# torgeiba/CPUPerformanceRayTracer

Measured on AMD Instinct MI355X. Metric: ray-samples/sec (pixels×spp×bounces) at 1920×1080; ms/frame, higher is better.
Workload: dtype f32; 1 GPU; c2_1080p; width=1920, height=1080, spp=8, bounces=8, parallelism=single GPU, step=one launch accumulating 8 frames (spp) of every pixel in HBM

## Files before the change

### cpuperformanceraytracer_amd/csrc/pt_chain.h

```cpp
#pragma once
#include <hip/hip_runtime.h>
#include <stdint.h>

#include "pt_kernel.h"
#include "pt_guard.h"
#include "pt_tile_queue.h"

__device__ __forceinline__ float pt_px_ld(const float* p)
{
    return __builtin_bit_cast(float, __hip_atomic_load(reinterpret_cast<uint32_t*>(const_cast<float*>(p)), __ATOMIC_RELAXED,
                                                       __HIP_MEMORY_SCOPE_AGENT));
}
__device__ __forceinline__ void pt_px_st(float* p, float v)
{
    __hip_atomic_store(reinterpret_cast<uint32_t*>(p), __builtin_bit_cast(uint32_t, v), __ATOMIC_RELAXED, __HIP_MEMORY_SCOPE_AGENT);
}

typedef unsigned pt_v3u __attribute__((ext_vector_type(3)));
typedef float pt_v3f __attribute__((ext_vector_type(3)));
constexpr int kPtCpolSc1 = 16;
constexpr int kPtBufRsrcWord3 = 0x00020000;
__device__ __forceinline__ void pt_px_ld3(const float* buf, uint32_t nbytes, size_t cs, size_t pi, float& x, float& y, float& z)
{
    if (cs == 1 && nbytes) {
        const __amdgpu_buffer_rsrc_t r = __builtin_amdgcn_make_buffer_rsrc(const_cast<float*>(buf), 0, (int)nbytes, kPtBufRsrcWord3);
        const pt_v3f v = __builtin_bit_cast(pt_v3f, __builtin_amdgcn_raw_buffer_load_b96(r, (int)(pi * 4u), 0, kPtCpolSc1));
        x = v.x, y = v.y, z = v.z;
        return;
    }
    x = pt_px_ld(buf + pi), y = pt_px_ld(buf + pi + cs), z = pt_px_ld(buf + pi + 2 * cs);
}
__device__ __forceinline__ void pt_px_st3(float* buf, uint32_t nbytes, size_t cs, size_t pi, float x, float y, float z)
{
    if (cs == 1 && nbytes) {
        const __amdgpu_buffer_rsrc_t r = __builtin_amdgcn_make_buffer_rsrc(buf, 0, (int)nbytes, kPtBufRsrcWord3);
        const pt_v3f v = {x, y, z};
        __builtin_amdgcn_raw_buffer_store_b96(__builtin_bit_cast(pt_v3u, v), r, (int)(pi * 4u), 0, kPtCpolSc1);
        return;
    }
    pt_px_st(buf + pi, x), pt_px_st(buf + pi + cs, y), pt_px_st(buf + pi + 2 * cs, z);
}
__device__ __forceinline__ uint32_t pt_px_nbytes(size_t floats)
{
    return floats * 4u < (1ull << 31) ? (uint32_t)(floats * 4u) : 0u;
}

__device__ __forceinline__ void pt_chain_started(unsigned long long* started)
{
    if (started && threadIdx.x == 0) __hip_atomic_fetch_add(started, 1ull, __ATOMIC_RELAXED, __HIP_MEMORY_SCOPE_SYSTEM);
}

__device__ __forceinline__ bool pt_chain_ready(const uint32_t* ep, uint32_t e, uint32_t w)
{
    const uint32_t t = pt_entry_tile(e), part = pt_entry_part(e);
    uint32_t m = ~0u;
    if (part != 2u) {
        const uint32_t a = __hip_atomic_load(const_cast<uint32_t*>(ep + 2u * t), __ATOMIC_RELAXED, __HIP_MEMORY_SCOPE_AGENT);
        m = a < m ? a : m;
    }
    if (part != 1u) {
        const uint32_t b = __hip_atomic_load(const_cast<uint32_t*>(ep + 2u * t + 1u), __ATOMIC_RELAXED, __HIP_MEMORY_SCOPE_AGENT);
        m = b < m ? b : m;
    }
    return __builtin_amdgcn_readfirstlane(m) >= w;
}

#ifndef PT_CHAIN_DIAG
#define PT_CHAIN_DIAG 0
#endif
constexpr uint32_t kPtChainPolls = PT_CHAIN_DIAG ? 1u << 16 : 1u << 21;
static __device__ uint32_t pt_chain_polls_dev = kPtChainPolls;
constexpr uint32_t kPtDiagWaves = 34, kPtDiagEnded = 35, kPtDiagWaiting = 36;
__device__ __forceinline__ unsigned* pt_chain_diag_prev(unsigned* q, uint32_t seq)
{
    return q - (size_t)(seq % 4u) * PT_QUEUE_WORDS + (size_t)((seq + 3u) % 4u) * PT_QUEUE_WORDS;
}
__device__ __forceinline__ void pt_chain_wait(const uint32_t* ep, uint32_t e, uint32_t w, uint32_t* err, int lane,
                                              unsigned* qdiag = nullptr)
{
    if (pt_chain_ready(ep, e, w)) return;
    bool ok = false;
    uint32_t polls = 0;
    if (PT_CHAIN_DIAG && qdiag && lane == 0) atomicAdd(qdiag + kPtDiagWaiting, 1u);
    do {
        __builtin_amdgcn_s_sleep(8);
        ok = pt_chain_ready(ep, e, w);
    } while (!ok && ++polls < pt_chain_polls_dev);
    if (PT_CHAIN_DIAG && qdiag && lane == 0) atomicSub(qdiag + kPtDiagWaiting, 1u);
#if PT_CHAIN_DIAG
    if (!ok && lane == 0 && qdiag) {
        unsigned* const qp = pt_chain_diag_prev(qdiag, w + 1u);
        auto rd = [](unsigned* p) { return __hip_atomic_fetch_add(p, 0u, __ATOMIC_RELAXED, __HIP_MEMORY_SCOPE_AGENT); };
        const uint32_t t = pt_entry_tile(e);
        printf("chain wait ran out: launch %u entry %u (tile %u) epochs %u %u | this launch: waves %u ended %u waiting %u "
               "| previous: waves %u ended %u waiting %u | block %u wave %u\n",
               w + 1u, e, t, rd(const_cast<uint32_t*>(ep + 2u * t)), rd(const_cast<uint32_t*>(ep + 2u * t + 1u)),
               rd(qdiag + kPtDiagWaves), rd(qdiag + kPtDiagEnded), rd(qdiag + kPtDiagWaiting), rd(qp + kPtDiagWaves),
               rd(qp + kPtDiagEnded), rd(qp + kPtDiagWaiting), blockIdx.x, threadIdx.x >> 6);
    }
#endif
    if (!ok && lane == 0) {
        const uint32_t t = pt_entry_tile(e), part = pt_entry_part(e);
        uint32_t m = ~0u;
        if (part != 2u) m = __hip_atomic_fetch_add(const_cast<uint32_t*>(ep + 2u * t), 0u, __ATOMIC_RELAXED, __HIP_MEMORY_SCOPE_AGENT);
        if (part != 1u) {
            const uint32_t b = __hip_atomic_fetch_add(const_cast<uint32_t*>(ep + 2u * t + 1u), 0u, __ATOMIC_RELAXED, __HIP_MEMORY_SCOPE_AGENT);
            m = b < m ? b : m;
        }
        const uint32_t behind = m >= w ? 0u : (w - m < 127u ? w - m : 127u);
        pt_guard_report(err, PT_G_CHAIN_WAIT, (t & 0xffffffu) | (behind << 24) | (m < w ? 0x80000000u : 0u));
    }
}

__device__ __forceinline__ void pt_chain_publish(uint32_t* ep, uint32_t e, uint32_t seq, uint32_t delay, int lane)
{
    if (__builtin_expect(delay != 0u, 0)) {
        const unsigned long long t0 = __builtin_amdgcn_s_memrealtime();
        while (__builtin_amdgcn_s_memrealtime() - t0 < 100ull * delay) __builtin_amdgcn_s_sleep(8);
    }
    asm volatile("s_waitcnt vmcnt(0)" ::: "memory");
    if (lane == 0) {
        const uint32_t t = pt_entry_tile(e), part = pt_entry_part(e);
        if (part != 2u) __hip_atomic_store(ep + 2u * t, seq, __ATOMIC_RELAXED, __HIP_MEMORY_SCOPE_AGENT);
        if (part != 1u) __hip_atomic_store(ep + 2u * t + 1u, seq, __ATOMIC_RELAXED, __HIP_MEMORY_SCOPE_AGENT);
    }
}
```

### cpuperformanceraytracer_amd/csrc/pt_guard.h

```cpp
#pragma once
#include <hip/hip_runtime.h>
#include <stdint.h>

#include "pt_kernel.h"

#ifndef PT_CHECKED
#define PT_CHECKED 0
#endif

__device__ __forceinline__ void pt_guard_report(uint32_t* err, uint32_t id, uint32_t detail)
{
    if (!err) return;
    atomicAdd(&err[PT_ERR_GUARD_COUNT], 1u);
    atomicMin(reinterpret_cast<unsigned long long*>(err + PT_ERR_GUARD_FIRST), ((unsigned long long)id << 32) | detail);
}

#define PT_GUARD(err, cond, id, detail) \
    (!PT_CHECKED || (cond) || (pt_guard_report((err), (uint32_t)(id), (uint32_t)(detail)), false))
```

### cpuperformanceraytracer_amd/csrc/pt_kernel.hip

```cpp
#include "pt_kernel.h"
#include "pt_exactmath.h"
#include "pt_sincosf.h"
#define PT_IT_HD __device__ __forceinline__
#define PT_IT_DIV(a, b) pt::div_guarded((a), (b))
#define PT_IT_SQRT(x) pt::sqrt_guarded(x)
#include "pt_invtrig.h"
#define PT_EC_HD __device__ __forceinline__
#define PT_EC_RCP(x) pt::rcp_rn(x)
#define PT_EC_DIV(a, b) pt::div_rn((a), (b), pt::rcp_rn(b))
#define PT_EC_SQRT(x) pt::sqrt_rn(x)
#include "pt_envcert.h"
#include "pt_tile_queue.h"
#include "pt_kernel_pick.h"
#include "pt_guard.h"
#include "pt_tonemap.h"
#include "pt_output.h"
#include "pt_wave.h"
#include "pt_chain.h"
#include <math.h>
#include <algorithm>
#include <utility>

namespace {

// ... 761 lines not shown
                    next_item += ntaken;
                }
                if ((live & ~idle) == 0 && ntaken == 0) break;
                ++tile_work;
                DIAG_ADD(1, t_it);
                DIAG_MARK(t_dir);
                if (COUNT) ++n_iter;
                bool queued = false;
                if (had || took) {
                    D = normalize(add(n, random_unit_vector(rng)));
                    DIAG_ADD(2, t_dir);
                    DIAG_MARK(t_tr);
                    const Hit h = trace<DemofoxScene, false, QV, SPHC>(s_axis, s_qv, P, D);
                    DIAG_ADD(3, t_tr);
                    DIAG_MARK(t_sh);
                    if (COUNT) ++n_seg, n_fb += (unsigned long long)h.fb;
                    bool done;
                    if (h.best == PT_SUPER_FAR) {
                        if (DEFER) queued = true;
                        else ret = add(ret, miss_radiance<ENV>(job, amb, D));
                        done = true;
                        if (COUNT) ++n_esc;
                    } else {
                        const PtLdsPrim pr = prim_at(s_prim, h.id);
                        n = hit_normal(pr, h, P, D);
                        P = add(add(P, mul(D, h.best)), mul(n, PT_NUDGE));
                        ret = add(ret, mulv(v3(pr.er, pr.eg, pr.eb), T));
                        T = mulv(T, v3(pr.ar, pr.ag, pr.ab));
                        bounce += 1;
                        done = bounce > B;
                    }
                    if (done) {
                        if (own && it_f == nf - 1) {
                            c_keep = ret;
                        } else {
                            lds_f32* c = col_lds + (it_lane * CHS + it_f) * 3;
                            c[0] = ret.x;
                            c[1] = ret.y;
                            c[2] = ret.z;
                        }
                        bounce = 0;
                    }
                    DIAG_ADD(4, t_sh);
                }
                if (DEFER) {
                    const uint64_t qm = pt_ballot(queued);
                    if (queued) {
                        const int r = __builtin_amdgcn_mbcnt_hi((uint32_t)(qm >> 32),
                                                               __builtin_amdgcn_mbcnt_lo((uint32_t)qm, 0u));
                        envq[qn + r] = make_float4(D.x, D.y, D.z, __builtin_bit_cast(float, (it_lane * CHS + it_f) * 3));
                    }
                    qn += __popcll(qm);
                    if (qn >= 64) {
                        qn -= 64;
                        drain(qn, 64);
                    }
                }
            }
            if (DEFER && qn > 0) drain(0, qn);
            if (f0 + CH >= S) next_tile = tq.next(job.err);
            DIAG_MARK(t_c);
            const int clc = txi * 8 + (lane & 7), clr = tyi * 8 + (lane >> 3);
            const bool cvalid = clc < job.ncols && clr < job.nrows && pt_part_has_lane(part, lane);
            if (cvalid) {
                if (!MULTI) {
                    const float* px = job.buf + out_index<LAYOUT>(job, clc, clr);
                    acc = v3(px[0], px[cs], px[2 * cs]);
                }
                for (int fi = 0; fi < nf; ++fi) {
                    V3 c = c_keep;
                    if (mine) {
                        if (own && fi == nf - 1) {
                            c = c_keep;
                        } else {
                            const lds_f32* cp = col_lds + (lane * CHS + fi) * 3;
                            c = v3(cp[0], cp[1], cp[2]);
                        }
                    }
                    const V3 colr = c;
                    const int f = f0 + fi;
                    const float t = WTAB && f < kMaxWeights ? s_w[f] : pt::rcp_rn((float)(job.frame_first + (uint32_t)f) + 1.0f);
                    acc = add(acc, mul(sub(colr, acc), t));
                }
            }
            DIAG_ADD(5, t_c);
        }
        }
        if (txi * 8 + (lane & 7) < job.ncols && tyi * 8 + (lane >> 3) < job.nrows && pt_part_has_lane(part, lane)) {
            float* px = job.buf + out_index<LAYOUT>(job, txi * 8 + (lane & 7), tyi * 8 + (lane >> 3));
            px[0] = acc.x;
            px[cs] = acc.y;
            px[2 * cs] = acc.z;
        }
        if (job.cost && lane == 0) pt_record_cost(job.cost, this_tile, total_tiles, tile_work);
        if (S <= 0) next_tile = tq.next(job.err);
        tile = __builtin_amdgcn_readfirstlane(next_tile);
#if PT_DIAG && !PT_DIAG_WAVES_ONLY
        if (job.counters && lane == 0 && n_tiles_diag <= 32) {
            unsigned long long* tl = job.counters + 32 + 4 * 65536 + 96 * (size_t)(blockIdx.x * kWavesPerBlock + wv);
            tl[3 * (n_tiles_diag - 1) + 0] = r_tile0;
            tl[3 * (n_tiles_diag - 1) + 1] = __builtin_amdgcn_s_memrealtime();
            tl[3 * (n_tiles_diag - 1) + 2] = ((unsigned long long)diag_tile_id << 32) | tile_work;
        }
#endif
        DIAG_ADD(6, t_tile);
    }
    tq.report(job.err);
    if (COUNT) {
        for (int off = 32; off > 0; off >>= 1) {
            n_seg += __shfl_xor(n_seg, off, 64);
            n_samp += __shfl_xor(n_samp, off, 64);
            n_esc += __shfl_xor(n_esc, off, 64);
            n_prim += __shfl_xor(n_prim, off, 64);
            n_fb += __shfl_xor(n_fb, off, 64);
            n_sky += __shfl_xor(n_sky, off, 64);
        }
        if (lane == 0) {
            atomicAdd(&job.counters[PT_CNT_SEGMENTS], n_seg);
            atomicAdd(&job.counters[PT_CNT_LANE_SLOTS], 64ull * n_iter);
            atomicAdd(&job.counters[PT_CNT_SAMPLES], n_samp);
            atomicAdd(&job.counters[PT_CNT_ESCAPED], n_esc);
            atomicAdd(&job.counters[PT_CNT_PRIMARY], n_prim);
            atomicAdd(&job.counters[PT_CNT_FALLBACK], n_fb);
            atomicAdd(&job.counters[PT_CNT_SKY], n_sky);
        }
    }
#if PT_DIAG
    if (job.counters && lane == 0) {
#if PT_DIAG >= 2
            for (int k = 0; k < 7; ++k) atomicAdd(&job.counters[PT_CNT_N + k], dg[k]);
#endif
            const unsigned long long r_death = __builtin_amdgcn_s_memrealtime();
#if !PT_DIAG_NOATOMIC
            const unsigned long long t_death = __builtin_amdgcn_s_memtime();
            atomicAdd(&job.counters[PT_CNT_N + 7], t_death - t_birth);
            atomicAdd(&job.counters[PT_CNT_N + 10], r_death - r_birth);
            atomicMax(&job.counters[PT_CNT_N + 8], r_birth);
            atomicMin(&job.counters[PT_CNT_N + 9], r_death);
            atomicMax(&job.counters[PT_CNT_N + 11], r_death);
            atomicMin(&job.counters[PT_CNT_N + 12], r_birth);
#endif
            unsigned long long* rec = job.counters + 32 + 4 * (size_t)(blockIdx.x * kWavesPerBlock + wv);
            rec[0] = r_birth;
            rec[1] = r_death;
            rec[2] = n_tiles_diag;
            rec[3] = n_iter;
    }
#endif
}

constexpr uint32_t kCtWaveFloats = 2u * 64u * (uint32_t)kChunk * 3u;
enum : int {
    kWsTcur, kWsHm, kWsHm1, kWsNh, kWsF0next, kWsF0A, kWsTD, kWsF0D, kWsNfD, kWsHmD, kWsHmD1,
    kWsTileSeg, kWsSegA, kWsSegD, kWsFlags, kWsChunks, kWsCamMode, kWsCam, kWsCam1, kWsWords
};

#ifndef PT_ENV_WAVES
#define PT_ENV_WAVES 6
#endif
#ifndef PT_ENV_Q
#define PT_ENV_Q 96
#endif
static_assert(PT_ENV_Q >= 64 && PT_ENV_Q <= 128, "the env miss queue holds 64 .. 128 entries per wave");
template <int LAYOUT, bool ENV, bool COUNT, bool PRESENT>
__device__ __forceinline__ void render_body_ct(const PtJob& job)
{
    pt_chain_started(job.started);
#if PT_CHAIN_DIAG
    if (job.tile_epoch && blockIdx.x == 0 && threadIdx.x == 0) job.queue[kPtDiagWaves] = gridDim.x * (blockDim.x / 64u);
#endif
    const PtScene* __restrict__ sc = job.scene;
    constexpr int kWavesPerBlock = waves_per_block<ENV>();
    constexpr bool QV = true;
    __shared__ PtLdsPrim s_prim[PT_NPRIMS];
    __shared__ AxisRow s_axis[PT_NQUADS * kAxisRowsPerQuad<true>];
    __shared__ float4 s_qv[kQuadVecs];
    __shared__ float s_w[kMaxWeights];
    __shared__ float4 s_rec[kWavesPerBlock][64];
    __shared__ float s_nrm[kWavesPerBlock][3][64];
    __shared__ float s_acc[kWavesPerBlock][3][64];
    __shared__ uint32_t s_seed[kWavesPerBlock][64];
    __shared__ uint32_t s_ws[kWavesPerBlock][kWsWords];
    __shared__ uint32_t s_tq[kWavesPerBlock][PtTileQueue<kWavesPerBlock>::kWords];
    constexpr int kQ = ENV ? PT_ENV_Q : 1;
    __shared__ float4 s_envq[ENV ? kWavesPerBlock : 1][kQ][2];
    {
        const int t = threadIdx.x;
        if (t < PT_NPRIMS) {
            PtLdsPrim e;
            if (t < PT_NQUADS) {
                e.nx = sc->qn[t][0]; e.ny = sc->qn[t][1]; e.nz = sc->qn[t][2];
            } else {
                e.nx = sc->sph[t - PT_NQUADS][0]; e.ny = sc->sph[t - PT_NQUADS][1]; e.nz = sc->sph[t - PT_NQUADS][2];
            }
            e.ar = sc->albedo[t][0]; e.ag = sc->albedo[t][1]; e.ab = sc->albedo[t][2];
            e.er = sc->emissive[t][0]; e.eg = sc->emissive[t][1]; e.eb = sc->emissive[t][2];
            e.pad0 = e.pad1 = e.pad2 = 0.0f;
            s_prim[t] = e;
        } else if (t >= 64 && t < 64 + PT_NQUADS * kAxisRowsPerQuad<true>) {
            constexpr int F = kAxisRowsPerQuad<true> / 3;
            const int r = (t - 64) / 3, k = (t - 64) % 3, q = r / F, fl = r % F;
            const auto vk = [&](int v) { return sc->qv[q][fl ? 3 - v : v][k]; };
            s_axis[t - 64] = AxisRow{vk(0), vk(1), vk(2), vk(3)};
        } else if (t >= 128 && t < 128 + kQuadVecs) {
            const int r = (t - 128) / 3, part = (t - 128) % 3, q = r >> 1, fl = r & 1;
            float e[4];
            for (int i = 0; i < 4; ++i) {
                const int f = part * 4 + i, v = f / 3, k = f % 3;
                e[i] = sc->qv[q][fl ? 3 - v : v][k];
            }
            s_qv[t - 128] = make_float4(e[0], e[1], e[2], e[3]);
        }
        if (t < kMaxWeights && t < job.nframes)
            s_w[t] = pt::rcp_rn((float)(job.frame_first + (uint32_t)t) + 1.0f);
    }
    __syncthreads();

    const int lane = threadIdx.x & 63;
    const int wv = __builtin_amdgcn_readfirstlane(threadIdx.x >> 6);
    const int tiles_x = (job.ncols + 7) >> 3;
    const uint32_t total_tiles = (uint32_t)tiles_x * (uint32_t)((job.nrows + 7) >> 3);
    const int S = job.nframes, B = job.num_bounces;
    const size_t cs = (LAYOUT == PT_LAYOUT_INTERLEAVED) ? 1u : 8u;
    float* const slots = job.ct_slots + (size_t)(blockIdx.x * kWavesPerBlock + wv) * kCtWaveFloats;
    if (!PT_GUARD(job.err, blockIdx.x * (uint32_t)kWavesPerBlock + (uint32_t)wv < job.ct_waves, PT_G_SLOT_BASE,
                  blockIdx.x * (uint32_t)kWavesPerBlock + (uint32_t)wv))
        return;
    const size_t px_extent = pixel_extent<LAYOUT>(job);
    const uint32_t pxb = pt_px_nbytes(px_extent);
    auto weight = [&](int f) {
        return f < kMaxWeights ? s_w[f] : pt::rcp_rn((float)(job.frame_first + (uint32_t)f) + 1.0f);
    };
    auto present = [&](int lc, int lr, const V3& acc) {
        if constexpr (PRESENT) {
            const size_t o = (size_t)lr * (uint32_t)job.ncols + (uint32_t)lc;
            if (PT_GUARD(job.err, o < (size_t)job.nrows * (uint32_t)job.ncols, PT_G_PIXOUT, o))
                job.pix_out[o] = pt_tone::pack<true, true>(acc.x, acc.y, acc.z, job.pix_xrgb != 0);
        }
    };

    Camera cam;
    cam.W = job.cam_W;
    cam.H = job.cam_H;
    cam.yW = job.cam_yW;
    cam.yH = job.cam_yH;
    cam.aspect = job.cam_aspect;
    cam.yAspect = job.cam_yAspect;
    cam.cam_dist = sc->cam_dist;
    const V3 amb = v3(sc->ambient[0], sc->ambient[1], sc->ambient[2]);
    const V3 zero = v3(0.0f, 0.0f, 0.0f), one = v3(1.0f, 1.0f, 1.0f);
    unsigned long long n_seg = 0, n_iter = 0, n_samp = 0, n_esc = 0, n_prim = 0, n_fb = 0, n_sky = 0, n_cam = 0;
#if PT_DIAG
    const unsigned long long r_birth = __builtin_amdgcn_s_memrealtime();
    unsigned long long n_tiles_diag = 0;
    uint32_t didx_cur = 0, didxA = 0, didxD = 0;
    unsigned long long* const dtl =
        job.counters ? job.counters + 32 + 4 * 65536 + 96 * (size_t)(blockIdx.x * kWavesPerBlock + wv) : nullptr;
#endif

    pt_queue_zero_next(job.queue_next);
    constexpr uint32_t kNone = PtTileQueue<kWavesPerBlock>::kNone;
    {
        PtTileQueue<kWavesPerBlock> q(job.queue, job.order, job.units, job.nunits, total_tiles, wv);
        q.back = (uint64_t)blockIdx.x * 100u >= (uint64_t)gridDim.x * (100u - (job.ct_back_pct < 100u ? job.ct_back_pct : 100u)) &&
                 job.ct_back_pct != 0;
        q.save(s_tq[wv], lane);
    }

    uint32_t* const ws = s_ws[wv];
    auto ws_ld = [&](int k) -> uint32_t { return __builtin_amdgcn_readfirstlane(ws[k]); };
    auto ws_st = [&](int k, uint32_t v) {
        if (lane == 0) ws[k] = v;
    };
    auto chain_wait_tile = [&](uint32_t e) {
        if (job.chain_wait != 0u) pt_chain_wait(job.tile_epoch, e, job.chain_wait, job.err, lane, PT_CHAIN_DIAG ? job.queue : nullptr);
    };
    auto chain_publish = [&](uint32_t e) {
        if (job.tile_epoch) pt_chain_publish(job.tile_epoch, e, job.chain_seq, job.chain_delay, lane);
    };

    if (lane == 0) {
        ws[kWsTcur] = kNone;
        ws[kWsFlags] = 0u;
        ws[kWsChunks] = 0u;
        ws[kWsTileSeg] = 0u;
        ws[kWsCamMode] = job.cam_mode;
        ws[kWsCam] = (uint32_t)(uintptr_t)job.cam_cache;
        ws[kWsCam1] = (uint32_t)((uintptr_t)job.cam_cache >> 32);
    }
    int cA = 0;
    int nfA = 0;
    uint32_t fterm = 0;
    int issA = 0, nitA = 0;
    bool hasD = false;
    uint64_t dmask = 0;
    uint32_t divA = 0;
    const uint32_t rec_cost = (job.cost || PT_DIAG) ? 0x80000000u : 0u;
    V3 P = zero, D = zero, T = zero, ret = zero, n = zero;
    uint32_t rng = 0;
    int bounce = 0;
    int it_addr = 0;

    auto start_chunk = [&]() {
        while (nitA == 0) {
            const int f0next = (int)ws_ld(kWsF0next);
            if (ws_ld(kWsTcur) != kNone && f0next < S) {
                fterm = __umul24(job.frame_first + (uint32_t)f0next, 26699u);
                nfA = S - f0next < kChunk ? S - f0next : kChunk;
                ws_st(kWsF0A, (uint32_t)f0next);
                ws_st(kWsF0next, (uint32_t)(f0next + nfA));
                divA = ((65536u + (uint32_t)nfA - 1u) / (uint32_t)nfA) | rec_cost;
                issA = 0;
                nitA = (int)ws_ld(kWsNh) * nfA;
                ws_st(kWsSegA, 0u);
#if PT_DIAG
                didxA = didx_cur;
#endif
                break;
            }
            ws_st(kWsTcur, kNone);
            const uint32_t flags = ws_ld(kWsFlags);
            if (flags & 2u) break;
            PtTileQueue<kWavesPerBlock> tq = PtTileQueue<kWavesPerBlock>::restore(s_tq[wv]);
            uint32_t tile = (flags & 1u) ? tq.next(job.err) : tq.first(job.err);
            tile = __builtin_amdgcn_readfirstlane(tile);
            tq.save(s_tq[wv], lane);
            ws_st(kWsFlags, tile == kNone ? 3u : 1u);
            if (tile == kNone) break;
            chain_wait_tile(tile);
#if PT_DIAG && !PT_DIAG_WAVES_ONLY
            didx_cur = (uint32_t)n_tiles_diag;
            if (dtl && lane == 0 && n_tiles_diag < 32) {
                dtl[3 * n_tiles_diag + 0] = __builtin_amdgcn_s_memrealtime();
                dtl[3 * n_tiles_diag + 2] = (unsigned long long)tile << 32;
                dtl[3 * n_tiles_diag + 1] = n_iter;
            }
#endif
#if PT_DIAG
            ++n_tiles_diag;
#endif
            const uint32_t part = pt_entry_part(tile);
            const int tyi = (int)(pt_entry_tile(tile) / (uint32_t)tiles_x), txi = (int)(pt_entry_tile(tile) % (uint32_t)tiles_x);
            const int lc = txi * 8 + (lane & 7), lr = tyi * 8 + (lane >> 3);
            const bool valid = lc < job.ncols && lr < job.nrows && pt_part_has_lane(part, lane);
            const float fx = (float)(job.col0 + lc);
            const float fy = (float)(job.height - 1 - (job.row_start + lr * job.row_stride));
            const V3 D0 = camera_dir(cam, fx, fy);
            const bool all_sky = pt_ballot(valid && !sky_ray(D0)) == 0;
            bool items = false;
            V3 P1 = zero, N1 = zero;
            int id1 = 0;
            if (valid) {
                const uint32_t ci = pt_entry_tile(tile) * 64u + (uint32_t)lane;
                const uint32_t cam_mode = ws_ld(kWsCamMode);
                unsigned long long* const cam_cache =
                    (unsigned long long*)(uintptr_t)((unsigned long long)ws_ld(kWsCam) | ((unsigned long long)ws_ld(kWsCam1) << 32));
                const bool cam_ok = cam_mode != PT_CAM_NONE && !all_sky &&
                                    PT_GUARD(job.err, ci < total_tiles * 64u, PT_G_CAM_INDEX, ci);
                Hit h{PT_SUPER_FAR, -1, 0, 0};
                if (!COUNT && cam_ok && cam_mode == PT_CAM_USE) {
                    const unsigned long long r = cam_cache[ci];
                    h.id = pt_cam_id(r);
                    h.best = h.id < 0 ? PT_SUPER_FAR : __builtin_bit_cast(float, pt_cam_best_bits(r));
                    h.flag = pt_cam_flag(r);
                    h.fb = pt_cam_fb(r);
                } else if (!all_sky) {
                    h = trace<DemofoxScene, true, QV, true>(s_axis, s_qv, zero, D0);
                    if (cam_ok) {
                        const unsigned long long r =
                            pt_cam_pack(__builtin_bit_cast(uint32_t, h.best), h.best == PT_SUPER_FAR ? -1 : h.id, h.flag, h.fb);
                        if (!COUNT && cam_mode == PT_CAM_FILL) cam_cache[ci] = r;
                        if (COUNT && cam_mode == PT_CAM_USE) {
                            ++n_cam;
                            if (cam_cache[ci] != r && !(h.best == PT_SUPER_FAR && pt_cam_id(cam_cache[ci]) < 0))
                                pt_guard_report(job.err, PT_G_CAM_RECORD, ci);
                        }
                    }
                }
                if (COUNT) ++n_seg, ++n_prim, n_fb += (unsigned long long)h.fb, n_sky += all_sky ? 1ull : 0ull;
                if (COUNT) n_samp += (unsigned long long)S;
                V3 c_keep;
                if (h.best == PT_SUPER_FAR) {
                    c_keep = add(zero, miss_radiance<ENV>(job, amb, D0));
                    if (COUNT) n_esc += (unsigned long long)S;
                } else {
                    const PtLdsPrim pr = prim_at(s_prim, h.id);
                    const V3 n1 = hit_normal(pr, h, zero, D0);
                    P1 = add(add(zero, mul(D0, h.best)), mul(n1, PT_NUDGE));
                    N1 = n1;
                    id1 = h.id;
                    items = B != 0;
                    c_keep = add(zero, mulv(v3(pr.er, pr.eg, pr.eb), one));
                }
                const size_t pi = out_index<LAYOUT>(job, lc, lr);
                if (!items && PT_GUARD(job.err, pi + 2 * cs < px_extent, PT_G_PIXEL, pi)) {
                    V3 acc;
                    pt_px_ld3(job.buf, pxb, cs, pi, acc.x, acc.y, acc.z);
                    for (int f = 0; f < S; ++f) acc = add(acc, mul(sub(c_keep, acc), weight(f)));
                    pt_px_st3(job.buf, pxb, cs, pi, acc.x, acc.y, acc.z);
                    present(lc, lr, acc);
                }
            }
            const uint64_t hm = pt_ballot(items);
            const int nh = __popcll(hm);
            if (nh == 0) {
                if (job.cost && lane == 0) pt_record_cost(job.cost, tile, total_tiles, 1u);
                chain_publish(tile);
#if PT_DIAG && !PT_DIAG_WAVES_ONLY
                if (dtl && lane == 0 && didx_cur < 32) {
                    dtl[3 * didx_cur + 1] = __builtin_amdgcn_s_memrealtime();
                    dtl[3 * didx_cur + 2] = ((unsigned long long)tile << 32) | 1u;
                }
#endif
                continue;
            }
            if (items) {
                const int slot = __builtin_amdgcn_mbcnt_hi((uint32_t)(hm >> 32), __builtin_amdgcn_mbcnt_lo((uint32_t)hm, 0u));
                s_rec[wv][slot] = make_float4(P1.x, P1.y, P1.z, __builtin_bit_cast(float, id1 | (lane << 8)));
                s_nrm[wv][0][slot] = N1.x;
                s_nrm[wv][1][slot] = N1.y;
                s_nrm[wv][2][slot] = N1.z;
                s_seed[wv][slot] = __umul24((uint32_t)(job.col0 + lc), 1973u) +
                                   __umul24((uint32_t)(job.height - 1 - (job.row_start + lr * job.row_stride)), 9277u);
            }
            ws_st(kWsTcur, tile);
            ws_st(kWsHm, (uint32_t)hm);
            ws_st(kWsHm + 1, (uint32_t)(hm >> 32));
            ws_st(kWsNh, (uint32_t)nh);
            ws_st(kWsF0next, 0u);
        }
    };
    int qn = 0;
    auto drain = [&](int q0, int m) {
        if (ENV && lane < m) {
            const float4 e = s_envq[ENV ? wv : 0][q0 + lane][0], r = s_envq[ENV ? wv : 0][q0 + lane][1];
            const V3 c = env_sample(job.env, job.env_w, job.env_h, v3(e.x, e.y, e.z));
            const uint32_t a = __builtin_bit_cast(uint32_t, e.w);
            if (PT_GUARD(job.err, a + 3u <= kCtWaveFloats, PT_G_ITEM_SLOT, a)) {
                float* const o = slots + a;
                o[0] = r.x + c.x;
                o[1] = r.y + c.y;
                o[2] = r.z + c.z;
            }
        }
    };
    auto fold_D = [&]() {
        if (ENV && qn > 0) {
            drain(0, qn);
            qn = 0;
        }
        const int c = cA ^ 1;
        __builtin_amdgcn_fence(__ATOMIC_RELEASE, "workgroup");
        __builtin_amdgcn_fence(__ATOMIC_ACQUIRE, "workgroup");
        const int f0D = (int)ws_ld(kWsF0D), nfD = (int)ws_ld(kWsNfD);
        const uint32_t tD = ws_ld(kWsTD);
        const uint64_t hmD = (uint64_t)ws_ld(kWsHmD) | ((uint64_t)ws_ld(kWsHmD + 1) << 32);
        const bool first = f0D == 0, last = f0D + nfD == S;
        if ((hmD >> lane) & 1u) {
            const float4* sp = (const float4*)(slots + (c * 64 + lane) * (kChunk * 3));
            float4 v[kChunk * 3 / 4];
#pragma unroll
            for (int i = 0; i < kChunk * 3 / 4; ++i)
                if (i * 4 < nfD * 3) v[i] = sp[i];
            const float* fr = (const float*)v;
            const uint32_t tdi = pt_entry_tile(tD);
            const int lc = (int)(tdi % (uint32_t)tiles_x) * 8 + (lane & 7), lr = (int)(tdi / (uint32_t)tiles_x) * 8 + (lane >> 3);
            size_t pi = out_index<LAYOUT>(job, lc, lr);
            if (!PT_GUARD(job.err, pi + 2 * cs < px_extent, PT_G_PIXEL, pi)) pi = 0;
            V3 acc;
            if (first) pt_px_ld3(job.buf, pxb, cs, pi, acc.x, acc.y, acc.z);
            else acc = v3(s_acc[wv][0][lane], s_acc[wv][1][lane], s_acc[wv][2][lane]);
#pragma unroll
            for (int f = 0; f < kChunk; ++f) {
                if (f < nfD) {
                    const V3 colr = v3(fr[3 * f], fr[3 * f + 1], fr[3 * f + 2]);
                    acc = add(acc, mul(sub(colr, acc), weight(f0D + f)));
                }
            }
            if (last) {
                pt_px_st3(job.buf, pxb, cs, pi, acc.x, acc.y, acc.z);
                present(lc, lr, acc);
            } else {
                s_acc[wv][0][lane] = acc.x;
                s_acc[wv][1][lane] = acc.y;
                s_acc[wv][2][lane] = acc.z;
            }
        }
        const uint32_t tile_seg = ws_ld(kWsTileSeg) + ws_ld(kWsSegD);
        ws_st(kWsTileSeg, last ? 0u : tile_seg);
        const uint32_t tile_cost = 1u + (tile_seg + 63u) / 64u;
        if (last) {
            if (job.cost && lane == 0) pt_record_cost(job.cost, tD, total_tiles, tile_cost);
            chain_publish(tD);
#if PT_DIAG && !PT_DIAG_WAVES_ONLY
            if (dtl && lane == 0 && didxD < 32) {
                const unsigned long long it0 = dtl[3 * didxD + 1];
                dtl[3 * didxD + 1] = __builtin_amdgcn_s_memrealtime();
                dtl[3 * didxD + 2] = ((unsigned long long)tD << 32) | tile_cost |
                                     ((n_iter - it0) << 16);
            }
#endif
        }
        hasD = false;
    };

    start_chunk();
    uint32_t idle_events = 0;
    bool fault = false;
    while (!fault) {
        bool event = false;
        if (hasD && dmask == 0) {
            fold_D();
            event = true;
        }
        if (nitA > 0 && issA >= nitA && !hasD) {
            ws_st(kWsTD, ws_ld(kWsTcur));
            ws_st(kWsHmD, ws_ld(kWsHm));
            ws_st(kWsHmD + 1, ws_ld(kWsHm + 1));
            ws_st(kWsF0D, ws_ld(kWsF0A));
            ws_st(kWsNfD, (uint32_t)nfA);
            hasD = true;
            dmask = pt_ballot(bounce != 0);
            ws_st(kWsSegD, ws_ld(kWsSegA));
#if PT_DIAG
            didxD = didxA;
#endif
            nitA = 0;
            issA = 0;
            cA ^= 1;
            const uint32_t n_chunks = ws_ld(kWsChunks) + 1u;
            ws_st(kWsChunks, n_chunks);
            if (__builtin_expect(n_chunks > job.guard_cap, 0)) {
                fault = true;
                break;
            }
            start_chunk();
            event = true;
            if (dmask == 0) continue;
        }
        if (nitA == 0 && !hasD) break;
        idle_events = event ? 0u : idle_events + 1u;
        if (__builtin_expect(idle_events > 2u, 0)) {
            fault = true;
            break;
        }
        while (true) {
            const bool had = bounce != 0;
            const uint64_t idle = pt_ballot(!had);
            bool took = false;
            int ntaken = 0;
            if (idle != 0 && issA < nitA) {
                const int rank = __builtin_amdgcn_mbcnt_hi((uint32_t)(idle >> 32), __builtin_amdgcn_mbcnt_lo((uint32_t)idle, 0u));
                const int k = issA + rank;
                const bool take = !had && k < nitA;
                took = take;
                const int slot_pm = take ? (int)(__umul24((uint32_t)k, divA) >> 16) : 0;
                const int fi = take ? k - (int)__umul24((uint32_t)slot_pm, (uint32_t)nfA) : 0;
                if (take) {
                    const float4 a0 = s_rec[wv][slot_pm];
                    const int packed = __builtin_bit_cast(int, a0.w);
                    const int sId = packed & 0xff;
                    const int src = packed >> 8;
                    const PtLdsPrim pr = prim_at(s_prim, sId);
                    rng = (s_seed[wv][slot_pm] + fterm + __umul24((uint32_t)fi, 26699u)) | 1u;
                    P = v3(a0.x, a0.y, a0.z);
                    n = v3(s_nrm[wv][0][slot_pm], s_nrm[wv][1][slot_pm], s_nrm[wv][2][slot_pm]);
                    ret = emissive0(pr);
                    T = mulv(one, v3(pr.ar, pr.ag, pr.ab));
                    bounce = 1;
                    it_addr = (int)__umul24((uint32_t)(cA * 64 + src), (uint32_t)(kChunk * 3)) + fi * 3;
                }
                const int npop = __popcll(idle);
                ntaken = npop < nitA - issA ? npop : nitA - issA;
                issA += ntaken;
            }
            if (idle == ~0ull && ntaken == 0) break;
            idle_events = 0;
            if (COUNT || PT_DIAG) ++n_iter;
            bool done = false, queued = false;
            if (had || took) {
                D = normalize(add(n, random_unit_vector(rng)));
                const Hit h = trace<DemofoxScene, false, QV, true>(s_axis, s_qv, P, D);
                if (COUNT) ++n_seg, n_fb += (unsigned long long)h.fb;
                if (h.best == PT_SUPER_FAR) {
                    if (ENV) queued = true;
                    else ret = add(ret, amb);
                    done = true;
                    if (COUNT) ++n_esc;
                } else {
                    const PtLdsPrim pr = prim_at(s_prim, h.id);
                    n = hit_normal(pr, h, P, D);
                    P = add(add(P, mul(D, h.best)), mul(n, PT_NUDGE));
                    ret = add(ret, mulv(v3(pr.er, pr.eg, pr.eb), T));
                    T = mulv(T, v3(pr.ar, pr.ag, pr.ab));
                    bounce += 1;
                    done = bounce > B;
                }
                if (done) {
                    if (!queued && PT_GUARD(job.err, (uint32_t)it_addr + 3u <= kCtWaveFloats, PT_G_ITEM_SLOT, it_addr)) {
                        float* c = slots + it_addr;
                        c[0] = ret.x;
                        c[1] = ret.y;
                        c[2] = ret.z;
                    }
                    bounce = 0;
                }
            }
            if (ENV) {
                const uint64_t qm = pt_ballot(queued);
                const int nq = __popcll(qm);
                if (kQ < 128 && qn + nq > kQ) {
                    drain(0, qn);
                    qn = 0;
                }
                if (queued && PT_GUARD(job.err, qn + nq <= kQ, PT_G_ENVQ, qn + nq)) {
                    const int r = __builtin_amdgcn_mbcnt_hi((uint32_t)(qm >> 32), __builtin_amdgcn_mbcnt_lo((uint32_t)qm, 0u));
                    s_envq[ENV ? wv : 0][qn + r][0] = make_float4(D.x, D.y, D.z, __builtin_bit_cast(float, it_addr));
                    s_envq[ENV ? wv : 0][qn + r][1] = make_float4(ret.x, ret.y, ret.z, 0.0f);
                }
                qn += nq;
                if (qn >= 64) {
                    qn -= 64;
                    drain(qn, 64);
                }
            }
            const uint64_t ended = pt_ballot(done);
            if ((int)divA < 0) {
                const int inD = __popcll(dmask), in_all = __popcll(pt_ballot(had || took));
                if (lane == 0) {
                    ws[kWsSegA] += (uint32_t)(in_all - inD);
                    ws[kWsSegD] += (uint32_t)inD;
                }
            }
            dmask &= ~ended;
            if (hasD && dmask == 0) break;
            if (nitA > 0 && issA >= nitA && !hasD) break;
        }
    }
    if (__builtin_expect(fault, 0) && lane == 0 && job.err) {
        atomicAdd(&job.err[0], 1u);
        atomicMin(&job.err[1], pt_entry_tile(nitA > 0 ? ws_ld(kWsTcur) : (hasD ? ws_ld(kWsTD) : 0u)));
    }
    PtTileQueue<kWavesPerBlock>::restore(s_tq[wv]).report(job.err);
#if PT_CHAIN_DIAG
    if (job.tile_epoch && lane == 0) atomicAdd(job.queue + kPtDiagEnded, 1u);
#endif
#if PT_DIAG
    if (job.counters && lane == 0) {
        unsigned long long* rec = job.counters + 32 + 4 * (size_t)(blockIdx.x * kWavesPerBlock + wv);
        rec[0] = r_birth;
        rec[1] = __builtin_amdgcn_s_memrealtime();
        rec[2] = n_tiles_diag;
        rec[3] = n_iter;
    }
#endif
    if (COUNT) {
        for (int off = 32; off > 0; off >>= 1) {
            n_seg += __shfl_xor(n_seg, off, 64);
            n_samp += __shfl_xor(n_samp, off, 64);
            n_esc += __shfl_xor(n_esc, off, 64);
            n_prim += __shfl_xor(n_prim, off, 64);
            n_fb += __shfl_xor(n_fb, off, 64);
            n_sky += __shfl_xor(n_sky, off, 64);
            n_cam += __shfl_xor(n_cam, off, 64);
        }
        if (lane == 0) {
            atomicAdd(&job.counters[PT_CNT_SEGMENTS], n_seg);
            atomicAdd(&job.counters[PT_CNT_LANE_SLOTS], 64ull * n_iter);
            atomicAdd(&job.counters[PT_CNT_SAMPLES], n_samp);
            atomicAdd(&job.counters[PT_CNT_ESCAPED], n_esc);
            atomicAdd(&job.counters[PT_CNT_PRIMARY], n_prim);
            atomicAdd(&job.counters[PT_CNT_FALLBACK], n_fb);
            atomicAdd(&job.counters[PT_CNT_SKY], n_sky);
            atomicAdd(&job.counters[PT_CNT_CAM_CHECKED], n_cam);
        }
    }
}

#ifndef PT_AMBIENT_WAVES
#define PT_AMBIENT_WAVES 5
#endif
template <int LAYOUT, bool COUNT, bool MULTI, bool RING>
__global__ __launch_bounds__(64 * waves_per_block<false>()) __attribute__((amdgpu_waves_per_eu(PT_AMBIENT_WAVES, PT_AMBIENT_WAVES))) void
pt_render_kernel(PtJob job)
{
    render_body<LAYOUT, false, COUNT, MULTI, RING>(job);
}

template <int LAYOUT, bool COUNT, bool MULTI>
__global__ __launch_bounds__(64 * waves_per_block<true>()) void pt_render_env_kernel(PtJob job)
{
    render_body<LAYOUT, true, COUNT, MULTI, false>(job);
}

template <int LAYOUT, bool COUNT, int WAVES, bool PRESENT = false>
__global__ __launch_bounds__(64 * waves_per_block<false>()) __attribute__((amdgpu_waves_per_eu(WAVES, WAVES))) void
pt_render_ct_kernel(PtJob job)
{
    render_body_ct<LAYOUT, false, COUNT, PRESENT>(job);
}

template <int LAYOUT, bool COUNT, bool PRESENT = false>
__global__ __launch_bounds__(64 * waves_per_block<true>()) __attribute__((amdgpu_waves_per_eu(PT_ENV_WAVES, PT_ENV_WAVES))) void pt_render_ct_env_kernel(PtJob job)
{
    render_body_ct<LAYOUT, true, COUNT, PRESENT>(job);
}

using PtKernel = void (*)(PtJob);
struct PtInstance {
    PtKey key;
    PtKernel kern;
};
template <int LAYOUT, bool ENV, bool COUNT, bool MULTI, bool RING, bool CT, bool WIDE, bool PRESENT>
constexpr PtInstance pt_instance()
{
    static_assert(!(ENV && (RING || WIDE)) && !(CT && (MULTI || RING)) && !(!CT && (WIDE || PRESENT)) && (MULTI || !RING));
    constexpr PtKey key{LAYOUT, ENV, COUNT, MULTI, RING, CT, WIDE, PRESENT};
    if constexpr (CT && ENV) return {key, pt_render_ct_env_kernel<LAYOUT, COUNT, PRESENT>};
    else if constexpr (CT) return {key, pt_render_ct_kernel<LAYOUT, COUNT, WIDE ? 6 : 5, PRESENT>};
    else if constexpr (ENV) return {key, pt_render_env_kernel<LAYOUT, COUNT, MULTI>};
    else return {key, pt_render_kernel<LAYOUT, COUNT, MULTI, RING>};
}
template <size_t... I>
constexpr PtKeyList<PtInstance, sizeof...(I)> pt_table(std::index_sequence<I...>)
{
    constexpr auto& k = kPtKeys.k;
    return {{pt_instance<k[I].layout, k[I].env, k[I].count, k[I].multi, k[I].ring, k[I].ct, k[I].wide, k[I].present>()...}};
}
constexpr auto kPtTable = pt_table(std::make_index_sequence<kPtKeyCount>{});
constexpr bool pt_table_matches()
{
    for (size_t i = 0; i < kPtKeyCount; ++i)
        if (!(kPtTable.k[i].key == kPtKeys.k[i])) return false;
    return true;
}
static_assert(kPtTable.size == kPtKeys.size && pt_table_matches(), "the table holds the listed keys, in their order");
static_assert(waves_per_block<false>() == kPickWaves && waves_per_block<true>() == kPickWaves && kChunk == kPickChunk &&
              PT_LAYOUT_TILED_PLANAR8 == kPickTiled, "pt_kernel_pick.h's constants");
PtResidentCache<kPtKeyCount> pt_resident;
int resident_of(int i) { return i < 0 ? 0 : pt_resident.get((size_t)i, (const void*)kPtTable.k[i].kern, 64 * kPickWaves); }

hipError_t launch_instance(int i, uint32_t grid, hipStream_t st, const PtJob& job)
{
    hipLaunchKernelGGL(kPtTable.k[i].kern, dim3(grid), dim3(64 * kPickWaves), 0, st, job);
    return hipGetLastError();
}

constexpr int kCostBins = 1024;
constexpr uint32_t kUnitCostMax = 12, kUnitCostMin = 2;
static_assert(kCostBins == 1024, "the schedule kernel scans one histogram bin per thread");

__device__ uint32_t block_exclusive_scan_1024(uint32_t* a, uint32_t* wave_tot)
{
    const uint32_t t = threadIdx.x, ln = t & 63, w = t >> 6;
    const uint32_t v = a[t];
    uint32_t x = v;
#pragma unroll
    for (int d = 1; d < 64; d <<= 1) {
        const uint32_t y = __shfl_up(x, d, 64);
        if (ln >= (uint32_t)d) x += y;
    }
    if (ln == 63) wave_tot[w] = x;
    __syncthreads();
    if (t == 0) {
        uint32_t run = 0;
        for (int k = 0; k < 16; ++k) {
            const uint32_t c = wave_tot[k];
            wave_tot[k] = run;
            run += c;
        }
        wave_tot[16] = run;
    }
    __syncthreads();
    a[t] = wave_tot[w] + x - v;
    const uint32_t total = wave_tot[16];
    __syncthreads();
    return total;
}

__global__ __launch_bounds__(1024) void pt_schedule_kernel(const uint32_t* __restrict__ cost, uint32_t* __restrict__ order,
                                                           uint32_t* __restrict__ units, uint32_t* __restrict__ nunits,
                                                           uint32_t n, uint32_t kUnitCost, uint32_t split_div,
                                                           uint32_t* err)
{
    __shared__ uint32_t hist[kCostBins];
    __shared__ uint32_t ucnt[kCostBins];
    __shared__ uint32_t wave_tot[17];
    __shared__ unsigned long long s_total;
    const uint32_t t = threadIdx.x;
    constexpr uint32_t nt = 1024, kBatch = 8;
    constexpr uint32_t kNoTile = 0xffffffffu;
    hist[t] = 0;
    if (t == 0) s_total = 0;
    __syncthreads();
    auto cost_at = [&](uint32_t i) { return i < n ? cost[i] + cost[n + i] : kNoTile; };
    auto bin_of = [&](uint32_t c) {
// ... 154 lines not shown
```

Measured before the change: 624.4 billion ray-samples/s.

## Stage job parameters in LDS and rematerialize them per event to cut live registers

```diff
diff --git a/cpuperformanceraytracer_amd/csrc/pt_chain.h b/cpuperformanceraytracer_amd/csrc/pt_chain.h
--- a/cpuperformanceraytracer_amd/csrc/pt_chain.h
+++ b/cpuperformanceraytracer_amd/csrc/pt_chain.h
@@ -75,6 +75,7 @@
 {
     return q - (size_t)(seq % 4u) * PT_QUEUE_WORDS + (size_t)((seq + 3u) % 4u) * PT_QUEUE_WORDS;
 }
+template <bool REPORT_HERE = false>
 __device__ __forceinline__ void pt_chain_wait(const uint32_t* ep, uint32_t e, uint32_t w, uint32_t* err, int lane,
                                               unsigned* qdiag = nullptr)
 {
@@ -108,7 +109,7 @@
             m = b < m ? b : m;
         }
         const uint32_t behind = m >= w ? 0u : (w - m < 127u ? w - m : 127u);
-        pt_guard_report(err, PT_G_CHAIN_WAIT, (t & 0xffffffu) | (behind << 24) | (m < w ? 0x80000000u : 0u));
+        pt_guard_report<REPORT_HERE>(err, PT_G_CHAIN_WAIT, (t & 0xffffffu) | (behind << 24) | (m < w ? 0x80000000u : 0u));
     }
 }
 
diff --git a/cpuperformanceraytracer_amd/csrc/pt_guard.h b/cpuperformanceraytracer_amd/csrc/pt_guard.h
--- a/cpuperformanceraytracer_amd/csrc/pt_guard.h
+++ b/cpuperformanceraytracer_amd/csrc/pt_guard.h
@@ -8,9 +8,11 @@
 #define PT_CHECKED 0
 #endif
 
+template <bool HERE = false>
 __device__ __forceinline__ void pt_guard_report(uint32_t* err, uint32_t id, uint32_t detail)
 {
     if (!err) return;
+    if (HERE) asm volatile("v_mov_b32 %0, %1" : "=v"(id) : "s"(id));
     atomicAdd(&err[PT_ERR_GUARD_COUNT], 1u);
     atomicMin(reinterpret_cast<unsigned long long*>(err + PT_ERR_GUARD_FIRST), ((unsigned long long)id << 32) | detail);
 }
diff --git a/cpuperformanceraytracer_amd/csrc/pt_kernel.hip b/cpuperformanceraytracer_amd/csrc/pt_kernel.hip
--- a/cpuperformanceraytracer_amd/csrc/pt_kernel.hip
+++ b/cpuperformanceraytracer_amd/csrc/pt_kernel.hip
@@ -937,8 +937,10 @@
 constexpr uint32_t kCtWaveFloats = 2u * 64u * (uint32_t)kChunk * 3u;
 enum : int {
     kWsTcur, kWsHm, kWsHm1, kWsNh, kWsF0next, kWsF0A, kWsTD, kWsF0D, kWsNfD, kWsHmD, kWsHmD1,
-    kWsTileSeg, kWsSegA, kWsSegD, kWsFlags, kWsChunks, kWsCamMode, kWsCam, kWsCam1, kWsWords
+    kWsTileSeg, kWsSegA, kWsSegD, kWsFlags, kWsChunks, kWsWords
 };
+static_assert(sizeof(PtJob) % 4 == 0, "PtJob is copied to LDS by words");
+constexpr int kJobWords = (int)(sizeof(PtJob) / 4), kJobCamDist = kJobWords;
 
 #ifndef PT_ENV_WAVES
 #define PT_ENV_WAVES 6
@@ -967,6 +969,7 @@
     __shared__ uint32_t s_seed[kWavesPerBlock][64];
     __shared__ uint32_t s_ws[kWavesPerBlock][kWsWords];
     __shared__ uint32_t s_tq[kWavesPerBlock][PtTileQueue<kWavesPerBlock>::kWords];
+    __shared__ uint32_t s_job[kJobWords + 1];
     constexpr int kQ = ENV ? PT_ENV_Q : 1;
     __shared__ float4 s_envq[ENV ? kWavesPerBlock : 1][kQ][2];
     {
@@ -998,40 +1001,57 @@
         }
         if (t < kMaxWeights && t < job.nframes)
             s_w[t] = pt::rcp_rn((float)(job.frame_first + (uint32_t)t) + 1.0f);
+        if (t < kJobWords) s_job[t] = reinterpret_cast<const uint32_t*>(&job)[t];
+        if (t == kJobCamDist) s_job[t] = __builtin_bit_cast(uint32_t, sc->cam_dist);
     }
     __syncthreads();
 
     const int lane = threadIdx.x & 63;
     const int wv = __builtin_amdgcn_readfirstlane(threadIdx.x >> 6);
-    const int tiles_x = (job.ncols + 7) >> 3;
-    const uint32_t total_tiles = (uint32_t)tiles_x * (uint32_t)((job.nrows + 7) >> 3);
-    const int S = job.nframes, B = job.num_bounces;
+    const int B = job.num_bounces;
     const size_t cs = (LAYOUT == PT_LAYOUT_INTERLEAVED) ? 1u : 8u;
     float* const slots = job.ct_slots + (size_t)(blockIdx.x * kWavesPerBlock + wv) * kCtWaveFloats;
     if (!PT_GUARD(job.err, blockIdx.x * (uint32_t)kWavesPerBlock + (uint32_t)wv < job.ct_waves, PT_G_SLOT_BASE,
                   blockIdx.x * (uint32_t)kWavesPerBlock + (uint32_t)wv))
         return;
-    const size_t px_extent = pixel_extent<LAYOUT>(job);
-    const uint32_t pxb = pt_px_nbytes(px_extent);
-    auto weight = [&](int f) {
-        return f < kMaxWeights ? s_w[f] : pt::rcp_rn((float)(job.frame_first + (uint32_t)f) + 1.0f);
+    struct Ev {
+        PtJob j;
+        Camera cam;
+        int S, tiles_x;
+        uint32_t total_tiles, pxb;
+        size_t px_extent;
     };
-    auto present = [&](int lc, int lr, const V3& acc) {
+    auto ev_args = [&]() {
+        uint32_t w[kJobWords];
+#pragma unroll
+        for (int i = 0; i < kJobWords; ++i) w[i] = __builtin_amdgcn_readfirstlane(s_job[i]);
+        Ev e;
+        __builtin_memcpy(&e.j, w, sizeof(PtJob));
+        e.cam.W = e.j.cam_W;
+        e.cam.H = e.j.cam_H;
+        e.cam.yW = e.j.cam_yW;
+        e.cam.yH = e.j.cam_yH;
+        e.cam.aspect = e.j.cam_aspect;
+        e.cam.yAspect = e.j.cam_yAspect;
+        e.cam.cam_dist = __builtin_bit_cast(float, (uint32_t)__builtin_amdgcn_readfirstlane(s_job[kJobCamDist]));
+        e.S = e.j.nframes;
+        e.tiles_x = (e.j.ncols + 7) >> 3;
+        e.total_tiles = (uint32_t)e.tiles_x * (uint32_t)((e.j.nrows + 7) >> 3);
+        e.px_extent = pixel_extent<LAYOUT>(e.j);
+        e.pxb = pt_px_nbytes(e.px_extent);
+        return e;
+    };
+    auto weight = [&](const Ev& ev, int f) {
+        return f < kMaxWeights ? s_w[f] : pt::rcp_rn((float)(ev.j.frame_first + (uint32_t)f) + 1.0f);
+    };
+    auto present = [&](const Ev& ev, int lc, int lr, const V3& acc) {
         if constexpr (PRESENT) {
-            const size_t o = (size_t)lr * (uint32_t)job.ncols + (uint32_t)lc;
-            if (PT_GUARD(job.err, o < (size_t)job.nrows * (uint32_t)job.ncols, PT_G_PIXOUT, o))
-                job.pix_out[o] = pt_tone::pack<true, true>(acc.x, acc.y, acc.z, job.pix_xrgb != 0);
+            const size_t o = (size_t)lr * (uint32_t)ev.j.ncols + (uint32_t)lc;
+            if (PT_GUARD(ev.j.err, o < (size_t)ev.j.nrows * (uint32_t)ev.j.ncols, PT_G_PIXOUT, o))
+                ev.j.pix_out[o] = pt_tone::pack<true, true>(acc.x, acc.y, acc.z, ev.j.pix_xrgb != 0);
         }
     };
 
-    Camera cam;
-    cam.W = job.cam_W;
-    cam.H = job.cam_H;
-    cam.yW = job.cam_yW;
-    cam.yH = job.cam_yH;
-    cam.aspect = job.cam_aspect;
-    cam.yAspect = job.cam_yAspect;
-    cam.cam_dist = sc->cam_dist;
     const V3 amb = v3(sc->ambient[0], sc->ambient[1], sc->ambient[2]);
     const V3 zero = v3(0.0f, 0.0f, 0.0f), one = v3(1.0f, 1.0f, 1.0f);
     unsigned long long n_seg = 0, n_iter = 0, n_samp = 0, n_esc = 0, n_prim = 0, n_fb = 0, n_sky = 0, n_cam = 0;
@@ -1046,6 +1066,7 @@
     pt_queue_zero_next(job.queue_next);
     constexpr uint32_t kNone = PtTileQueue<kWavesPerBlock>::kNone;
     {
+        const uint32_t total_tiles = (uint32_t)((job.ncols + 7) >> 3) * (uint32_t)((job.nrows + 7) >> 3);
         PtTileQueue<kWavesPerBlock> q(job.queue, job.order, job.units, job.nunits, total_tiles, wv);
         q.back = (uint64_t)blockIdx.x * 100u >= (uint64_t)gridDim.x * (100u - (job.ct_back_pct < 100u ? job.ct_back_pct : 100u)) &&
                  job.ct_back_pct != 0;
@@ -1057,11 +1078,12 @@
     auto ws_st = [&](int k, uint32_t v) {
         if (lane == 0) ws[k] = v;
     };
-    auto chain_wait_tile = [&](uint32_t e) {
-        if (job.chain_wait != 0u) pt_chain_wait(job.tile_epoch, e, job.chain_wait, job.err, lane, PT_CHAIN_DIAG ? job.queue : nullptr);
+    auto chain_wait_tile = [&](const Ev& ev, uint32_t e) {
+        if (ev.j.chain_wait != 0u)
+            pt_chain_wait<true>(ev.j.tile_epoch, e, ev.j.chain_wait, ev.j.err, lane, PT_CHAIN_DIAG ? ev.j.queue : nullptr);
     };
-    auto chain_publish = [&](uint32_t e) {
-        if (job.tile_epoch) pt_chain_publish(job.tile_epoch, e, job.chain_seq, job.chain_delay, lane);
+    auto chain_publish = [&](const Ev& ev, uint32_t e) {
+        if (ev.j.tile_epoch) pt_chain_publish(ev.j.tile_epoch, e, ev.j.chain_seq, ev.j.chain_delay, lane);
     };
 
     if (lane == 0) {
@@ -1069,9 +1091,6 @@
         ws[kWsFlags] = 0u;
         ws[kWsChunks] = 0u;
         ws[kWsTileSeg] = 0u;
-        ws[kWsCamMode] = job.cam_mode;
-        ws[kWsCam] = (uint32_t)(uintptr_t)job.cam_cache;
-        ws[kWsCam1] = (uint32_t)((uintptr_t)job.cam_cache >> 32);
     }
     int cA = 0;
     int nfA = 0;
@@ -1088,9 +1107,12 @@
 
     auto start_chunk = [&]() {
         while (nitA == 0) {
+            const Ev ev = ev_args();
+            const int S = ev.S, tiles_x = ev.tiles_x;
+            const uint32_t total_tiles = ev.total_tiles;
             const int f0next = (int)ws_ld(kWsF0next);
             if (ws_ld(kWsTcur) != kNone && f0next < S) {
-                fterm = __umul24(job.frame_first + (uint32_t)f0next, 26699u);
+                fterm = __umul24(ev.j.frame_first + (uint32_t)f0next, 26699u);
                 nfA = S - f0next < kChunk ? S - f0next : kChunk;
                 ws_st(kWsF0A, (uint32_t)f0next);
                 ws_st(kWsF0next, (uint32_t)(f0next + nfA));
@@ -1107,12 +1129,12 @@
             const uint32_t flags = ws_ld(kWsFlags);
             if (flags & 2u) break;
             PtTileQueue<kWavesPerBlock> tq = PtTileQueue<kWavesPerBlock>::restore(s_tq[wv]);
-            uint32_t tile = (flags & 1u) ? tq.next(job.err) : tq.first(job.err);
+            uint32_t tile = (flags & 1u) ? tq.next(ev.j.err) : tq.first(ev.j.err);
             tile = __builtin_amdgcn_readfirstlane(tile);
             tq.save(s_tq[wv], lane);
             ws_st(kWsFlags, tile == kNone ? 3u : 1u);
             if (tile == kNone) break;
-            chain_wait_tile(tile);
+            chain_wait_tile(ev, tile);
 #if PT_DIAG && !PT_DIAG_WAVES_ONLY
             didx_cur = (uint32_t)n_tiles_diag;
             if (dtl && lane == 0 && n_tiles_diag < 32) {
@@ -1127,21 +1149,20 @@
             const uint32_t part = pt_entry_part(tile);
             const int tyi = (int)(pt_entry_tile(tile) / (uint32_t)tiles_x), txi = (int)(pt_entry_tile(tile) % (uint32_t)tiles_x);
             const int lc = txi * 8 + (lane & 7), lr = tyi * 8 + (lane >> 3);
-            const bool valid = lc < job.ncols && lr < job.nrows && pt_part_has_lane(part, lane);
-            const float fx = (float)(job.col0 + lc);
-            const float fy = (float)(job.height - 1 - (job.row_start + lr * job.row_stride));
-            const V3 D0 = camera_dir(cam, fx, fy);
+            const bool valid = lc < ev.j.ncols && lr < ev.j.nrows && pt_part_has_lane(part, lane);
+            const float fx = (float)(ev.j.col0 + lc);
+            const float fy = (float)(ev.j.height - 1 - (ev.j.row_start + lr * ev.j.row_stride));
+            const V3 D0 = camera_dir(ev.cam, fx, fy);
             const bool all_sky = pt_ballot(valid && !sky_ray(D0)) == 0;
             bool items = false;
             V3 P1 = zero, N1 = zero;
             int id1 = 0;
             if (valid) {
                 const uint32_t ci = pt_entry_tile(tile) * 64u + (uint32_t)lane;
-                const uint32_t cam_mode = ws_ld(kWsCamMode);
-                unsigned long long* const cam_cache =
-                    (unsigned long long*)(uintptr_t)((unsigned long long)ws_ld(kWsCam) | ((unsigned long long)ws_ld(kWsCam1) << 32));
+                const uint32_t cam_mode = ev.j.cam_mode;
+                unsigned long long* const cam_cache = ev.j.cam_cache;
                 const bool cam_ok = cam_mode != PT_CAM_NONE && !all_sky &&
-                                    PT_GUARD(job.err, ci < total_tiles * 64u, PT_G_CAM_INDEX, ci);
+                                    PT_GUARD(ev.j.err, ci < total_tiles * 64u, PT_G_CAM_INDEX, ci);
                 Hit h{PT_SUPER_FAR, -1, 0, 0};
                 if (!COUNT && cam_ok && cam_mode == PT_CAM_USE) {
                     const unsigned long long r = cam_cache[ci];
@@ -1158,7 +1179,7 @@
                         if (COUNT && cam_mode == PT_CAM_USE) {
                             ++n_cam;
                             if (cam_cache[ci] != r && !(h.best == PT_SUPER_FAR && pt_cam_id(cam_cache[ci]) < 0))
-                                pt_guard_report(job.err, PT_G_CAM_RECORD, ci);
+                                pt_guard_report(ev.j.err, PT_G_CAM_RECORD, ci);
                         }
                     }
                 }
@@ -1166,7 +1187,7 @@
                 if (COUNT) n_samp += (unsigned long long)S;
                 V3 c_keep;
                 if (h.best == PT_SUPER_FAR) {
-                    c_keep = add(zero, miss_radiance<ENV>(job, amb, D0));
+                    c_keep = add(zero, miss_radiance<ENV>(ev.j, amb, D0));
                     if (COUNT) n_esc += (unsigned long long)S;
                 } else {
                     const PtLdsPrim pr = prim_at(s_prim, h.id);
@@ -1177,20 +1198,20 @@
                     items = B != 0;
                     c_keep = add(zero, mulv(v3(pr.er, pr.eg, pr.eb), one));
                 }
-                const size_t pi = out_index<LAYOUT>(job, lc, lr);
-                if (!items && PT_GUARD(job.err, pi + 2 * cs < px_extent, PT_G_PIXEL, pi)) {
+                const size_t pi = out_index<LAYOUT>(ev.j, lc, lr);
+                if (!items && PT_GUARD(ev.j.err, pi + 2 * cs < ev.px_extent, PT_G_PIXEL, pi)) {
                     V3 acc;
-                    pt_px_ld3(job.buf, pxb, cs, pi, acc.x, acc.y, acc.z);
-                    for (int f = 0; f < S; ++f) acc = add(acc, mul(sub(c_keep, acc), weight(f)));
-                    pt_px_st3(job.buf, pxb, cs, pi, acc.x, acc.y, acc.z);
-                    present(lc, lr, acc);
+                    pt_px_ld3(ev.j.buf, ev.pxb, cs, pi, acc.x, acc.y, acc.z);
+                    for (int f = 0; f < S; ++f) acc = add(acc, mul(sub(c_keep, acc), weight(ev, f)));
+                    pt_px_st3(ev.j.buf, ev.pxb, cs, pi, acc.x, acc.y, acc.z);
+                    present(ev, lc, lr, acc);
                 }
             }
             const uint64_t hm = pt_ballot(items);
             const int nh = __popcll(hm);
             if (nh == 0) {
-                if (job.cost && lane == 0) pt_record_cost(job.cost, tile, total_tiles, 1u);
-                chain_publish(tile);
+                if (ev.j.cost && lane == 0) pt_record_cost(ev.j.cost, tile, total_tiles, 1u);
+                chain_publish(ev, tile);
 #if PT_DIAG && !PT_DIAG_WAVES_ONLY
                 if (dtl && lane == 0 && didx_cur < 32) {
                     dtl[3 * didx_cur + 1] = __builtin_amdgcn_s_memrealtime();
@@ -1205,8 +1226,8 @@
                 s_nrm[wv][0][slot] = N1.x;
                 s_nrm[wv][1][slot] = N1.y;
                 s_nrm[wv][2][slot] = N1.z;
-                s_seed[wv][slot] = __umul24((uint32_t)(job.col0 + lc), 1973u) +
-                                   __umul24((uint32_t)(job.height - 1 - (job.row_start + lr * job.row_stride)), 9277u);
+                s_seed[wv][slot] = __umul24((uint32_t)(ev.j.col0 + lc), 1973u) +
+                                   __umul24((uint32_t)(ev.j.height - 1 - (ev.j.row_start + lr * ev.j.row_stride)), 9277u);
             }
             ws_st(kWsTcur, tile);
             ws_st(kWsHm, (uint32_t)hm);
@@ -1234,6 +1255,8 @@
             drain(0, qn);
             qn = 0;
         }
+        const Ev ev = ev_args();
+        const int S = ev.S, tiles_x = ev.tiles_x;
         const int c = cA ^ 1;
         __builtin_amdgcn_fence(__ATOMIC_RELEASE, "workgroup");
         __builtin_amdgcn_fence(__ATOMIC_ACQUIRE, "workgroup");
@@ -1250,33 +1273,35 @@
             const float* fr = (const float*)v;
             const uint32_t tdi = pt_entry_tile(tD);
             const int lc = (int)(tdi % (uint32_t)tiles_x) * 8 + (lane & 7), lr = (int)(tdi / (uint32_t)tiles_x) * 8 + (lane >> 3);
-            size_t pi = out_index<LAYOUT>(job, lc, lr);
-            if (!PT_GUARD(job.err, pi + 2 * cs < px_extent, PT_G_PIXEL, pi)) pi = 0;
+            size_t pi = out_index<LAYOUT>(ev.j, lc, lr);
+            if (!PT_GUARD(ev.j.err, pi + 2 * cs < ev.px_extent, PT_G_PIXEL, pi)) pi = 0;
+            int la;
+            asm volatile("v_mov_b32 %0, %1" : "=v"(la) : "v"(lane));
             V3 acc;
-            if (first) pt_px_ld3(job.buf, pxb, cs, pi, acc.x, acc.y, acc.z);
-            else acc = v3(s_acc[wv][0][lane], s_acc[wv][1][lane], s_acc[wv][2][lane]);
+            if (first) pt_px_ld3(ev.j.buf, ev.pxb, cs, pi, acc.x, acc.y, acc.z);
+            else acc = v3(s_acc[wv][0][la], s_acc[wv][1][la], s_acc[wv][2][la]);
 #pragma unroll
             for (int f = 0; f < kChunk; ++f) {
                 if (f < nfD) {
                     const V3 colr = v3(fr[3 * f], fr[3 * f + 1], fr[3 * f + 2]);
-                    acc = add(acc, mul(sub(colr, acc), weight(f0D + f)));
+                    acc = add(acc, mul(sub(colr, acc), weight(ev, f0D + f)));
                 }
             }
             if (last) {
-                pt_px_st3(job.buf, pxb, cs, pi, acc.x, acc.y, acc.z);
-                present(lc, lr, acc);
+                pt_px_st3(ev.j.buf, ev.pxb, cs, pi, acc.x, acc.y, acc.z);
+                present(ev, lc, lr, acc);
             } else {
-                s_acc[wv][0][lane] = acc.x;
-                s_acc[wv][1][lane] = acc.y;
-                s_acc[wv][2][lane] = acc.z;
+                s_acc[wv][0][la] = acc.x;
+                s_acc[wv][1][la] = acc.y;
+                s_acc[wv][2][la] = acc.z;
             }
         }
         const uint32_t tile_seg = ws_ld(kWsTileSeg) + ws_ld(kWsSegD);
         ws_st(kWsTileSeg, last ? 0u : tile_seg);
         const uint32_t tile_cost = 1u + (tile_seg + 63u) / 64u;
         if (last) {
-            if (job.cost && lane == 0) pt_record_cost(job.cost, tD, total_tiles, tile_cost);
-            chain_publish(tD);
+            if (ev.j.cost && lane == 0) pt_record_cost(ev.j.cost, tD, ev.total_tiles, tile_cost);
+            chain_publish(ev, tD);
 #if PT_DIAG && !PT_DIAG_WAVES_ONLY
             if (dtl && lane == 0 && didxD < 32) {
                 const unsigned long long it0 = dtl[3 * didxD + 1];
@@ -1315,7 +1340,7 @@
             cA ^= 1;
             const uint32_t n_chunks = ws_ld(kWsChunks) + 1u;
             ws_st(kWsChunks, n_chunks);
-            if (__builtin_expect(n_chunks > job.guard_cap, 0)) {
+            if (__builtin_expect(n_chunks > ev_args().j.guard_cap, 0)) {
                 fault = true;
                 break;
             }
@@ -1422,11 +1447,12 @@
             if (nitA > 0 && issA >= nitA && !hasD) break;
         }
     }
-    if (__builtin_expect(fault, 0) && lane == 0 && job.err) {
-        atomicAdd(&job.err[0], 1u);
-        atomicMin(&job.err[1], pt_entry_tile(nitA > 0 ? ws_ld(kWsTcur) : (hasD ? ws_ld(kWsTD) : 0u)));
-    }
-    PtTileQueue<kWavesPerBlock>::restore(s_tq[wv]).report(job.err);
+    uint32_t* const err = ev_args().j.err;
+    if (__builtin_expect(fault, 0) && lane == 0 && err) {
+        atomicAdd(&err[0], 1u);
+        atomicMin(&err[1], pt_entry_tile(nitA > 0 ? ws_ld(kWsTcur) : (hasD ? ws_ld(kWsTD) : 0u)));
+    }
+    PtTileQueue<kWavesPerBlock>::restore(s_tq[wv]).report(err);
 #if PT_CHAIN_DIAG
     if (job.tile_epoch && lane == 0) atomicAdd(job.queue + kPtDiagEnded, 1u);
 #endif
```

Result: no change. 623.7 billion ray-samples/s, median of 2 (-0.1%).
